# NYXFLOWER/GripNet

Measured on AMD Instinct MI355X. Metric: edges aggregated/sec, GripNet forward on pose-0, higher is better.
Workload: dtype f32

## Files before the change

gripnet_amd/_hip.py:

```python
from __future__ import annotations

import ctypes as C
import operator
import os
import threading

import torch

from ._cache import MISS, VersionedCache

_LIB_PATH = os.environ.get("GN_HIP_LIBRARY") or os.path.join(os.path.dirname(os.path.abspath(__file__)), "lib",
                                                            "libgripnet_hip.so")
_lib = None
_lock = threading.Lock()

GN_OK, GN_ERR_INVALID_ARG, GN_ERR_HIP, GN_ERR_INDEX_RANGE, GN_ERR_UNSUPPORTED, GN_ERR_EDGE_COUNT = range(6)
GN_RGCN_PARTIAL, GN_RGCN_ARITH_FAST, GN_RGCN_BASIS_TRANSPOSED = 1, 4, 64
GN_RGCN_PATH_SHIFT = 8
RGCN_PATHS = {"auto": 0, "pair": 1, "lds": 3, "general": 4, "table": 5}
GN_GEMM_RELU, GN_GEMM_ARITH_FAST, GN_GEMM_B_TRANSPOSED, GN_GEMM_ACCUMULATE, GN_GEMM_A_TRANSPOSED, GN_GEMM_JOIN_BATCH, GN_GEMM_OUT_BF16 = 1, 2, 4, 8, 16, 32, 64
GN_DM_TYPES_SORTED = 1
GN_DM_TYPE_TASKS = 2
ABI_VERSION = 165

_p, _i64, _int, _sz = C.c_void_p, C.c_int64, C.c_int, C.c_size_t

SIGNATURES = {
    "gn_version": (_int, []),
    "gn_last_error": (C.c_char_p, []),
    "gn_time_next_launch": (_int, [_p, _p]),
    "gn_host_scratch_release": (_sz, []),
    "gn_device_blocks_live": (_i64, []),
    "gn_time_launch_pending": (_int, []),
    "gn_gcn_plan_create": (_int, [_p, _p, _p, _i64, _i64, _int, _p, C.POINTER(_p)]),
    "gn_bipartite_plan_create": (_int, [_p, _p, _p, _i64, _i64, _i64, _p, C.POINTER(_p)]),
    "gn_sum_plan_create": (_int, [_p, _p, _p, _i64, _i64, _i64, _p, C.POINTER(_p)]),
    "gn_graph_plan_destroy": (None, [_p]),
    "gn_graph_plan_input_edges": (_i64, [_p]),
    "gn_graph_plan_nnz": (_i64, [_p]),
    "gn_graph_plan_export": (_int, [_p, _p, _p, _p]),
    "gn_graph_aggregate_f32": (_int, [_p, _p, _i64, _i64, _p, _i64, _p, _int, _p, _i64, _p, _p, _p]),
    "gn_split_planes_bytes": (_sz, [_i64, _int]),
    "gn_split_planes_f32": (_int, [_p, _i64, _i64, _i64, _i64, _p, _p]),
    "gn_transform_fusable": (_int, [_i64, _i64]),
    "gn_graph_transform_fusable": (_int, [_p, _i64, _i64]),
    "gn_graph_plan_build_blocked": (_int, [_p, _i64, _p]),
    "gn_graph_plan_blocked_cols": (_i64, [_p]),
    "gn_graph_plan_blocked_gather_kernel": (_int, [_p]),
    "gn_graph_plan_blocked_waves": (_i64, [_p, _p, _i64]),
    "gn_graph_blocked_applicable": (_int, [_p, _p, _i64, _i64, _p, _i64, _p, _p, _i64]),
    "gn_graph_chain_applicable": (_int, [_p, _p, _p, _i64, _i64, _p, _i64, _p, _p, _i64, _p]),
    "gn_graph_aggregate_chain_f32": (_int, [_p, _p, _p, _i64, _i64, _p, _i64, _p, _int, _p, _i64, _p, _p]),
    "gn_graph_gather_chained_f32": (_int, [_p, _p, _i64, _p]),
    "gn_graph_aggregate_tail_f32": (_int, [_p, _p, _i64, _i64, _p, _i64, _p, _int, _p, _i64, _p, _p, _p, _p, _int, _p]),
    "gn_graph_plan_build_transpose": (_int, [_p, _p]),
    "gn_graph_aggregate_t_f32": (_int, [_p, _p, _i64, _i64, _p, _i64, _p]),
    "gn_xtg_wide_supported": (_int, [_i64, _i64, _i64]),
    "gn_gemm_f32": (_int, [_p, _i64, _i64, _p, _i64, _p, _i64, _i64, _p, _i64, _i64, _i64, _i64, _i64, _i64, _p, _int, _p]),
    "gn_gemm_addend_f32": (_int, [_p, _i64, _i64, _p, _i64, _p, _i64, _i64, _p, _i64, _i64, _i64, _i64, _i64, _i64, _p, _p, _i64, _int, _p]),
    "gn_merge_f32": (_int, [_p, _i64, _p, _i64, _p, _i64, _i64, _i64, _int, _p]),
    "gn_softmax_rows_f32": (_int, [_p, _i64, _i64, _i64, _p]),
    "gn_softmax_rows_backward_f32": (_int, [_p, _i64, _p, _i64, _p, _i64, _i64, _i64, _p]),
    "gn_class_scores_f32": (_int, [_p, _i64, _i64, _p, _i64, _p, _i64, _i64, _i64, _int, _p, _i64, _p]),
    "gn_rgcn_plan_create": (_int, [_p, _p, _p, _int, _i64, _i64, _i64, _i64, _i64, _p, C.POINTER(_p)]),
    "gn_rgcn_plan_create_ex": (_int, [_p, _p, _p, _int, _i64, _i64, _i64, _i64, _i64, _int, _p, C.POINTER(_p)]),
    "gn_rgcn_plan_destroy": (None, [_p]),
    "gn_rgcn_plan_input_edges": (_i64, [_p]),
    "gn_rgcn_workspace_bytes": (_sz, [_p, _i64, _i64, _i64, _int]),
    "gn_rgcn_forward_path": (_int, [_p, _i64, _i64, _i64, _int]),
    "gn_rgcn_forward_choice": (_int, [_p, _p, _i64, _i64, _i64, _i64, _int, C.POINTER(_sz)]),
    "gn_cast_bf16": (_int, [_p, _i64, _p, _i64, _i64, _i64, _p]),
    "gn_graph_aggregate_bf16": (_int, [_p, _p, _i64, _i64, _p, _int, _p, _i64, _p, _p]),
    "gn_rgcn_forward_f32": (_int, [_p, _p, _i64, _i64, _p, _p, _i64, _p, _p, _i64, _int, _int, _p, _i64, _p, _p, _p, _sz, _p]),
    "gn_rgcn_finalize_f32": (_int, [_p, _p, _i64, _p, _i64, _i64, _p, _p, _i64, _int, _p, _i64, _p, _p]),
    "gn_distmult_forward_f32": (_int, [_p, _i64, _i64, _i64, _p, _p, _p, _p, _i64, _i64, _i64, _int, _p, _p, _p]),
    "gn_distmult_packed_forward_f32": (_int, [_p, _i64, _i64, _i64, _p, _p, _p, _i64, _i64, _i64, _int, _p, _p, _p]),
    "gn_distmult_plan_create": (_int, [_p, _p, _p, _i64, _i64, _i64, _i64, _p, C.POINTER(_p)]),
    "gn_distmult_plan_destroy": (None, [_p]),
    "gn_distmult_plan_edges": (_i64, [_p]),
    "gn_distmult_plan_forward_f32": (_int, [_p, _p, _i64, _i64, _p, _i64, _int, _p, _p]),
    "gn_distmult_plan_forward_cols_f32": (_int, [_p, _p, _i64, _i64, _i64, _i64, _p, _i64, _int, _p, _p]),
    "gn_xtg_workspace_bytes": (_sz, [_i64, _i64]),
    "gn_xtg_f32": (_int, [_p, _i64, _p, _i64, _i64, _i64, _i64, _p, _i64, _p, _sz, _int, _p]),
    "gn_distmult_backward_workspace_bytes": (_sz, [_i64, _i64, _i64, _i64]),
    "gn_dense_batch_begin": (_int, []),
    "gn_dense_batch_end": (_int, [_p]),
    "gn_distmult_type_tasks_bytes": (_sz, [_i64, _i64]),
# ... 608 lines not shown

    @property
    def nnz(self) -> int:
        return int(load().gn_graph_plan_nnz(self._h))

    def export(self):
        if self._export is None:
            n = self.nnz
            ei = torch.empty((2, n), dtype=torch.int64, device=self.device)
            nrm = torch.empty((n,), dtype=torch.float32, device=self.device)
            check(load().gn_graph_plan_export(self._h, ptr(ei), ptr(nrm), stream_ptr(self.device)))
            self._export = (ei, nrm)
        return self._export

    def __iter__(self):
        return iter(self.export())

    def aggregate(self, xw: torch.Tensor, bias, relu: bool, out: torch.Tensor, side=None, weight=None, planes=None, tail=None):
        sc = side_copy(side)
        pd = None
        if planes is not None:
            pd = planes[0].desc(planes[1], planes[2])
            planes[0].generation += 1
        if tail is not None:
            _call("gn_graph_aggregate_tail_f32", self._h, ptr(xw), ld(xw), xw.shape[1], ptr(weight), weight.shape[1], ptr(bias),
                  int(bool(relu)), ptr(out), ld(out), _ref(sc), _ref(pd), ptr(tail[0]), ptr(tail[1]), 1, stream_ptr(xw.device),
                  tag="gn_graph_aggregate_tail_f32[{}]".format(self.kind))
            return out
        _call("gn_graph_aggregate_f32", self._h, ptr(xw), ld(xw), xw.shape[1], ptr(weight),
              0 if weight is None else weight.shape[1], ptr(bias), int(bool(relu)),
              ptr(out), ld(out), _ref(sc), _ref(pd), stream_ptr(xw.device), tag="gn_graph_aggregate_f32[{}]".format(self.kind))
        return out

    def chain_ok(self, nxt: "GraphPlan", x: torch.Tensor, weight: torch.Tensor, bias, out: torch.Tensor, out_next: torch.Tensor) -> bool:
        return bool(load().gn_graph_chain_applicable(self._h, nxt._h, x.data_ptr(), ld(x), x.shape[1], weight.data_ptr(),
                                                     weight.shape[1], None if bias is None else bias.data_ptr(),
                                                     out.data_ptr(), ld(out), out_next.data_ptr()))

    def aggregate_chain(self, nxt: "GraphPlan", x: torch.Tensor, weight: torch.Tensor, bias, relu: bool, out: torch.Tensor, side=None):
        sc = side_copy(side)
        _call("gn_graph_aggregate_chain_f32", self._h, nxt._h, ptr(x), ld(x), x.shape[1], ptr(weight), weight.shape[1], ptr(bias),
              int(bool(relu)), ptr(out), ld(out), _ref(sc), stream_ptr(x.device))
        return out

    def gather_chained(self, out: torch.Tensor):
        _call("gn_graph_gather_chained_f32", self._h, ptr(out), ld(out), stream_ptr(out.device))
        return out

    def aggregate_bf16(self, xw: torch.Tensor, bias, relu: bool, out: torch.Tensor, side=None):
        if xw.dtype == torch.bfloat16:
            table = xw
        else:
            table = torch.empty(xw.shape, dtype=torch.bfloat16, device=xw.device)
            _call("gn_cast_bf16", ptr(xw), ld(xw), ptr(table), ld(table), xw.shape[0], xw.shape[1], stream_ptr(xw.device))
        sc = side_copy(side)
        _call("gn_graph_aggregate_bf16", self._h, ptr(table), ld(table), xw.shape[1], ptr(bias), int(bool(relu)),
              ptr(out), ld(out), _ref(sc), stream_ptr(xw.device), tag="gn_graph_aggregate_bf16[{}]".format(self.kind))
        return out

    def aggregate_t(self, g: torch.Tensor, out: torch.Tensor):
        if not getattr(self, "_has_t", False):
            check(load().gn_graph_plan_build_transpose(self._h, stream_ptr(g.device)))
            self._has_t = True
        _call("gn_graph_aggregate_t_f32", self._h, ptr(g), ld(g), g.shape[1], ptr(out), ld(out), stream_ptr(g.device))
        return out

# ... 709 lines not shown
```

gripnet_amd/csrc/aggregate.cuh:

```cuda
#pragma once

#include "common.h"

#ifndef GN_AGG_U
#define GN_AGG_U 2
#endif
#ifndef GN_AGG_U_WIDE
#define GN_AGG_U_WIDE 8
#endif
#ifndef GN_AGG_GRID
#define GN_AGG_GRID (256 * 8)
#endif

#ifndef GN_AGG_SHORT_MAX_DEG
#define GN_AGG_SHORT_MAX_DEG 8
#endif
#ifndef GN_AGG_GROUP_MAX_DEG
#define GN_AGG_GROUP_MAX_DEG 48
#endif
#ifndef GN_AGG_GROUP_U
#define GN_AGG_GROUP_U 8
#endif
#ifndef GN_MFMA_U16
#define GN_MFMA_U16 4
// ... 1 lines not shown

namespace gn {

struct AggArgs {
    const int32_t* rowptr;
    const uint32_t* col;
    const float* coef;
    const float* table;
    int64_t ld_table;
    int features;
    const float* rowdiv;
    const float* addend;
    int64_t ld_addend;
    const float* bias;
    int relu;
    float* out;
    int64_t ld_out;
    int rows;
    gn_side_copy side = {nullptr, 0, nullptr, 0, 0, 0, 0};
    gn_split_planes split = {nullptr, 0, 0, 0, 0};
    const uint32_t* ell_col = nullptr;
    const float* ell_coef = nullptr;
    int64_t nnz = -1;
    int64_t table_rows = -1;
    const uint16_t* table_bf16 = nullptr;
};

struct AggTail {
    const float* w;
    const float* b;
    int relu;
};

__device__ __forceinline__ void side_copy_stream(gn_side_copy s, int64_t thread, int64_t n_threads) {
    if (s.dst) {
        const int64_t total = s.rows * s.cols;
        for (int64_t t = thread; t < total; t += n_threads) {
            const int64_t i = t / s.cols, c = t - i * s.cols;
            const float v = s.src[i * s.ld_src + c];
            s.dst[i * s.ld_dst + c] = s.mode ? fabsf(v) : v;
        }
    }
}

inline int lanes_per_row(int64_t units) {
    int lpe = 1;
    while (lpe < units && lpe < kWave) lpe <<= 1;
    return lpe;
}

inline gn_status check_side(const gn_side_copy* side, int64_t rows, gn_side_copy* out) {
    *out = gn_side_copy{nullptr, 0, nullptr, 0, 0, 0, 0};
    if (!side || side->rows == 0 || side->cols == 0) return GN_OK;
    GN_REQUIRE(side->src && side->dst && side->rows > 0 && side->cols > 0, "side copy has a null pointer or a negative size");
    GN_REQUIRE(side->rows <= rows, "side copy has %lld rows, the launch only %lld", (long long)side->rows, (long long)rows);
    GN_REQUIRE(side->ld_src >= side->cols && side->ld_dst >= side->cols, "side copy leading dimension smaller than its row");
    GN_REQUIRE(side->mode == 0 || side->mode == 1, "unknown side copy mode %d", side->mode);
    *out = *side;
    return GN_OK;
}

inline bool transform_fusable(int64_t fin, int64_t fout) {
    if (fast_paths_disabled()) return false;
    return (fout == 16 && (fin == 16 || fin == 32 || fin == 64)) || (fout == 32 && (fin == 32 || fin == 64));
}

inline bool mfma_fusable(int64_t fin, int64_t fout, int64_t rows, int64_t nnz) {
    if (fast_paths_disabled()) return false;
    if (!(fin == 64 || fin == 128) || fout % 16 != 0 || fout < fin || fout > 128) return false;
    return nnz >= 0 && nnz < GN_AGG_GROUP_MAX_DEG * rows && rows >= 4096;
}

inline bool quad_gather_disabled() {
    const char* e = getenv("GN_DISABLE_QUAD");
    return e && e[0] == '1';
}

inline bool transform_takes_quad_kernel(int64_t fin, int64_t fout) { return fin == 16 && fout == 16 && !quad_gather_disabled(); }

inline bool lds_table_disabled() {
    const char* e = getenv("GN_DISABLE_LDS_TABLE");
    return e && e[0] == '1';
}

gn_status launch_aggregate(const AggArgs& a, hipStream_t st);
gn_status launch_aggregate_bf16(const AggArgs& a, int lpe, bool by_group, hipStream_t st);
gn_status launch_aggregate_transform(const AggArgs& a, const float* w, int fout, hipStream_t st);
gn_status launch_aggregate_transform_tail(const AggArgs& a, const float* w, int fout, const AggTail& tail, hipStream_t st);
gn_status launch_aggregate_mfma(const AggArgs& a, const float* w, int fout, hipStream_t st);
gn_status launch_split_planes(const float* src, int64_t ld_src, int64_t rows, int cols, int col0, const gn_split_planes& sp, hipStream_t st);

}
```

gripnet_amd/csrc/aggregate.hip:

```cpp
#include "aggregate.cuh"

#include <type_traits>

namespace gn {
namespace {

typedef float f32x4 __attribute__((ext_vector_type(4)));
typedef uint32_t u32x4 __attribute__((ext_vector_type(4)));

struct RowScalar {
    static constexpr int N = 1;
    static constexpr bool kMean = true;
    typedef float elem;
    typedef float raw;
    static __device__ __forceinline__ const elem* table(const AggArgs& a) { return a.table; }
    static __device__ __forceinline__ raw load(const elem* p) { return *p; }
    static __device__ __forceinline__ void add(float (&acc)[N], float coef, raw r) { acc[0] += coef * r; }
};
struct RowF32 {
    static constexpr int N = 4;
    static constexpr bool kMean = true;
    typedef float elem;
    typedef f32x4 raw;
    static __device__ __forceinline__ const elem* table(const AggArgs& a) { return a.table; }
// ... 176 lines not shown
                vv[u] = __shfl(v, t0 + u, LPE);
                r[u] = typename Row::raw{};
                if (t0 + u < cnt && active) r[u] = Row::load(tab + (int64_t)cc * a.ld_table);
            }
#pragma unroll
            for (int u = 0; u < U; ++u) Row::add(acc, vv[u], r[u]);
        }
    }
}

template <typename Row, int LPE, int U>
__global__ __launch_bounds__(256) void k_aggregate_group(AggArgs a) {
    constexpr int S = kWave / LPE, N = Row::N;
    const int lane = threadIdx.x & 63, slot = lane / LPE, j = lane % LPE;
    const int wave = (int)((blockIdx.x * (int64_t)blockDim.x + threadIdx.x) >> 6);
    const int fcol = N * j;
    const bool active = fcol < a.features;
    side_copy_stream(a.side, blockIdx.x * (int64_t)blockDim.x + threadIdx.x, (int64_t)gridDim.x * blockDim.x);
    const int row = wave * S + slot;
    const bool live = row < a.rows;
    const int begin = live ? a.rowptr[row] : 0, end = live ? a.rowptr[row + 1] : 0;
    float acc[N];
#pragma unroll
    for (int t = 0; t < N; ++t) acc[t] = 0.f;
    gather_group_row<Row, LPE, U>(a, Row::table(a) + fcol, begin, end, j, active, acc);
    if (live && active) finish_row<Row::kMean>(a, row, fcol, acc);
}

template <int CTRL>
__device__ __forceinline__ float tail_bcast(float v) {
    return __int_as_float(__builtin_amdgcn_mov_dpp(__float_as_int(v), CTRL, 0xf, 0xf, true));
}

template <int LPE, int FOUT, bool TAIL>
__device__ __forceinline__ void aggregate_transform(const AggArgs& a, const float* __restrict__ w, const AggTail& tail) {
    constexpr int FIN = 4 * LPE, S = kWave / LPE, G = kWave / FOUT, KPL = FIN / G;
    static_assert(KPL % 4 == 0, "K slice per lane must cover whole float4 groups");
    static_assert(!TAIL || LPE == 16, "the deferred tail transform is the last quad of a 16-lane group");
    const int lane = threadIdx.x & 63;
    const int slot = lane / LPE, j = lane % LPE;
    const int c = lane % FOUT, kq = lane / FOUT;
    const int block = blockIdx.x, n_blocks = gridDim.x;
    const int wave = (int)((block * (int64_t)blockDim.x + threadIdx.x) >> 6);
    const int n_waves = (int)(((int64_t)n_blocks * blockDim.x) >> 6);
    float wreg[KPL];
#pragma unroll
    for (int i = 0; i < KPL; ++i) wreg[i] = w[(kq * KPL + i) * FOUT + c];
    const float bias = a.bias ? a.bias[c] : 0.f;
    f32x4 tw[TAIL ? 16 : 1], tb = (f32x4){0.f, 0.f, 0.f, 0.f};
    if constexpr (TAIL) {
#pragma unroll
        for (int k = 0; k < 16; ++k) tw[k] = *reinterpret_cast<const f32x4*>(tail.w + 16 * k + 4 * (j & 3));
        if (tail.b) tb = *reinterpret_cast<const f32x4*>(tail.b + 4 * (j & 3));
    }

    const int64_t side_total = a.side.dst ? a.side.rows * a.side.cols : 0;
    const int64_t side_t0 = block * (int64_t)blockDim.x + threadIdx.x;
    float side_first = 0.f;
    if (side_t0 < side_total) {
        const int64_t i = side_t0 / a.side.cols, cc = side_t0 - i * a.side.cols;
        side_first = a.side.src[i * a.side.ld_src + cc];
    }
    for (int row = wave; row < a.rows; row += n_waves) {
        int begin, end;
        uint32_t cl0 = 0u;
        float v0 = 0.f;
        if (a.ell_col) {
            cl0 = a.ell_col[(size_t)row * 64 + lane];
            v0 = a.ell_coef[(size_t)row * 64 + lane];
            begin = 0;
            end = __popcll(__ballot(cl0 != 0xffffffffu));
            if (lane >= end) cl0 = 0u;
        } else {
            begin = a.rowptr[row];
            end = a.rowptr[row + 1];
        }
        float acc[4] = {0.f, 0.f, 0.f, 0.f};
        for (int base = begin; base < end; base += kWave) {
            const int mine = base + lane;
            const uint32_t cl = a.ell_col ? cl0 : (mine < end ? a.col[mine] : 0u);
            const float v = a.ell_col ? v0 : (mine < end ? (a.coef ? a.coef[mine] : 1.0f) : 0.f);
            const int cnt = min(kWave, end - base);
            constexpr int IT = kWave / S, UW = LPE >= 16 ? GN_AGG_U_WIDE : GN_AGG_U, U = IT < UW ? IT : UW;
            for (int it0 = 0; it0 * S < cnt; it0 += U) {
                float4 t[U];
                float vv[U];
#pragma unroll
                for (int it = 0; it < U; ++it) {
                    const int idx = (it0 + it) * S + slot;
                    const uint32_t cc = (uint32_t)__shfl((int)cl, idx);
                    vv[it] = __shfl(v, idx);
                    t[it] = make_float4(0.f, 0.f, 0.f, 0.f);
                    if (idx < cnt) t[it] = *reinterpret_cast<const float4*>(a.table + (int64_t)cc * a.ld_table + 4 * j);
                }
                if constexpr (TAIL) {
#pragma unroll
                    for (int it = 0; it < U; ++it) {
                        if ((it0 + it) * S >= cnt) continue;
                        const float g[4] = {t[it].x, t[it].y, t[it].z, t[it].w};
                        f32x4 h = tb;
#pragma unroll
                        for (int cc = 0; cc < 4; ++cc) {
                            h += tail_bcast<0x00>(g[cc]) * tw[cc];
                            h += tail_bcast<0x55>(g[cc]) * tw[4 + cc];
                            h += tail_bcast<0xAA>(g[cc]) * tw[8 + cc];
                            h += tail_bcast<0xFF>(g[cc]) * tw[12 + cc];
                        }
                        if (tail.relu) {
#pragma unroll
                            for (int cc = 0; cc < 4; ++cc) h[cc] = fmaxf(h[cc], 0.f);
                        }
                        if (j >= 12 && (it0 + it) * S + slot < cnt) t[it] = make_float4(h[0], h[1], h[2], h[3]);
                    }
                }
#pragma unroll
                for (int it = 0; it < U; ++it) {
                    acc[0] += vv[it] * t[it].x; acc[1] += vv[it] * t[it].y; acc[2] += vv[it] * t[it].z; acc[3] += vv[it] * t[it].w;
                }
            }
        }
#pragma unroll
        for (int off = LPE; off < kWave; off <<= 1) {
#pragma unroll
            for (int t = 0; t < 4; ++t) acc[t] += __shfl_xor(acc[t], off);
        }
        float part = 0.f;
#pragma unroll
        for (int i = 0; i < KPL; ++i) part += __shfl(acc[i % 4], kq * (KPL / 4) + i / 4) * wreg[i];
#pragma unroll
        for (int off = FOUT; off < kWave; off <<= 1) part += __shfl_xor(part, off);
        if (kq == 0) {
            float val = part + bias;
            if (a.relu) val = fmaxf(val, 0.f);
            a.out[(int64_t)row * a.ld_out + c] = val;
            if (a.split.planes) write_split(a.split, row, a.split.col_main + c, val);
        }
    }
    for (int64_t t = side_t0; t < side_total; t += (int64_t)n_blocks * blockDim.x) {
        const int64_t i = t / a.side.cols, cc = t - i * a.side.cols;
        const float v = t == side_t0 ? side_first : a.side.src[i * a.side.ld_src + cc];
        const float o = a.side.mode ? fabsf(v) : v;
        a.side.dst[i * a.side.ld_dst + cc] = o;
        if (a.split.planes) write_split(a.split, i, a.split.col_side + (int)cc, o);
    }
}

template <int LPE, int FOUT>
__global__ __launch_bounds__(256) void k_aggregate_transform(AggArgs a, const float* __restrict__ w) {
    aggregate_transform<LPE, FOUT, false>(a, w, AggTail{nullptr, nullptr, 0});
}
__global__ __launch_bounds__(256) void k_aggregate_transform_tail(AggArgs a, const float* __restrict__ w, AggTail tail) {
    aggregate_transform<16, 16, true>(a, w, tail);
}


template <int CTRL>
__device__ __forceinline__ int agg_dpp(int x) { return __builtin_amdgcn_mov_dpp(x, CTRL, 0xf, 0xf, true); }
template <int CTRL>
__device__ __forceinline__ float agg_dpp_add(float x) {
    return x + __int_as_float(__builtin_amdgcn_update_dpp(0, __float_as_int(x), CTRL, 0xf, 0xf, false));
}

template <int VPL>
__global__ __launch_bounds__(256) void k_aggregate_transform_q(AggArgs a, const float* __restrict__ w) {
    constexpr int FOUT = 16;
    const int lane = threadIdx.x & 63;
    const int q = lane >> 2, j = lane & 3;
    const int wave = (int)((blockIdx.x * (int64_t)blockDim.x + threadIdx.x) >> 6);
    const int n_waves = (int)(((int64_t)gridDim.x * blockDim.x) >> 6);
    f32x4 wreg[VPL];
#pragma unroll
    for (int v = 0; v < VPL; ++v)
#pragma unroll
        for (int c = 0; c < 4; ++c) wreg[v][c] = w[(16 * v + 4 * j + c) * FOUT + q];
    const float bias = a.bias ? a.bias[q] : 0.f;

    side_copy_stream(a.side, blockIdx.x * (int64_t)blockDim.x + threadIdx.x, (int64_t)gridDim.x * blockDim.x);
    const float* __restrict__ tab = a.table + 4 * j;
    for (int row = wave; row < a.rows; row += n_waves) {
        const int begin = a.rowptr[row], end = a.rowptr[row + 1];
        f32x4 s[VPL];
#pragma unroll
        for (int v = 0; v < VPL; ++v) s[v] = (f32x4){0.f, 0.f, 0.f, 0.f};
        for (int base = begin; base < end; base += kWave) {
            const int mine = base + lane;
// ... 250 lines not shown
}

gn_status launch_aggregate_transform(const AggArgs& a, const float* w, int fout, hipStream_t st) {
    if (a.rows == 0) return GN_OK;
    const int grid = (int)std::min<int64_t>(ceil_div(a.rows, 4), GN_AGG_GRID);
    const int key = a.features * 100 + fout;
    if (key == 1616 && a.ld_table % 4 == 0 && aligned16(a.table) && !quad_gather_disabled()) {
        k_aggregate_transform_q<1><<<grid, 256, 0, st>>>(a, w);
        GN_LAUNCH_CHECK();
        return GN_OK;
    }
    switch (key) {
        case 1616: k_aggregate_transform<4, 16><<<grid, 256, 0, st>>>(a, w); break;
        case 3216: k_aggregate_transform<8, 16><<<grid, 256, 0, st>>>(a, w); break;
        case 6416: k_aggregate_transform<16, 16><<<grid, 256, 0, st>>>(a, w); break;
        case 3232: k_aggregate_transform<8, 32><<<grid, 256, 0, st>>>(a, w); break;
        case 6432: k_aggregate_transform<16, 32><<<grid, 256, 0, st>>>(a, w); break;
        default: return fail(GN_ERR_UNSUPPORTED, "no fused transform for %d -> %d features", a.features, fout);
    }
    GN_LAUNCH_CHECK();
    return GN_OK;
}

gn_status launch_aggregate_transform_tail(const AggArgs& a, const float* w, int fout, const AggTail& tail, hipStream_t st) {
    if (a.features != 64 || fout != 16)
        return fail(GN_ERR_UNSUPPORTED, "the deferred tail transform exists for 64 -> 16 features, got %d -> %d", a.features, fout);
    if (a.rows == 0) return GN_OK;
    const int grid = (int)std::min<int64_t>(ceil_div(a.rows, 4), GN_AGG_GRID);
    k_aggregate_transform_tail<<<grid, 256, 0, st>>>(a, w, tail);
    GN_LAUNCH_CHECK();
    return GN_OK;
}

gn_status launch_aggregate(const AggArgs& a, hipStream_t st) {
    if (a.rows == 0 || a.features == 0) return GN_OK;
    const bool vec = (a.features % 4 == 0) && (a.ld_table % 4 == 0) && (a.ld_out % 4 == 0) && aligned16(a.table) &&
                     aligned16(a.out);
    const int lpe = lanes_per_row(vec ? a.features / 4 : a.features);
    if (vec && lpe >= 4 && lpe <= 16 && a.nnz > 0 && a.nnz < 8 * (int64_t)a.rows && a.rows >= 65536 && !a.coef && !a.rowdiv &&
        !a.addend && !a.bias && !a.relu && !a.side.dst && a.table_rows > 0 &&
        (size_t)a.table_rows * a.features * sizeof(float) <= 128 * 1024 && !fast_paths_disabled() && !lds_table_disabled()) {
        const size_t lds = (size_t)(a.table_rows + 1) * a.features * sizeof(float);
        const int wgs = (int)std::min<int64_t>(256, ceil_div((int64_t)a.rows * lpe, 2 * 1024));
        gn_status ls = GN_OK;
        dispatch_lpe<16, 4>(lpe, [&](auto l) {
            ls = allow_large_lds(reinterpret_cast<const void*>(k_aggregate_lds_table<decltype(l)::value>), 160 * 1024);
            if (ls == GN_OK) k_aggregate_lds_table<decltype(l)::value><<<wgs, 1024, lds, st>>>(a);
        });
        if (ls != GN_OK) return ls;
    } else if (vec && lpe <= 16 && a.nnz >= 0 && a.nnz < GN_AGG_SHORT_MAX_DEG * (int64_t)a.rows && !fast_paths_disabled()) {
        const int sgrid = (int)std::min<int64_t>(ceil_div((int64_t)a.rows * lpe, 256), GN_AGG_GRID);
        dispatch_lpe<16>(lpe, [&](auto l) { k_aggregate_short<decltype(l)::value><<<sgrid, 256, 0, st>>>(a); });
    } else if (vec && lpe <= 32 && a.nnz >= 0 && a.nnz < GN_AGG_GROUP_MAX_DEG * (int64_t)a.rows && !fast_paths_disabled()) {
        launch_group_per_row<RowF32>(a, lpe, st);
    } else if (vec) {
        launch_wave_per_row<RowF32>(a, lpe, st);
    } else {
        launch_wave_per_row<RowScalar>(a, lpe, st);
    }
    GN_LAUNCH_CHECK();
    return GN_OK;
}

gn_status launch_aggregate_bf16(const AggArgs& a, int lpe, bool by_group, hipStream_t st) {
    if (by_group) launch_group_per_row<RowBf16>(a, lpe, st); else launch_wave_per_row<RowBf16>(a, lpe, st);
    GN_LAUNCH_CHECK();
// ... 5 lines not shown
```

gripnet_amd/csrc/graph.hip:

```cpp
#include "aggregate.cuh"

bool gn_blocked_applicable(const gn_graph_plan* plan, const float* x, int64_t ld_x, int64_t fin, const float* w, int64_t fout,
                           const float* bias, const float* out, int64_t ld_out);
gn_status gn_blocked_aggregate(const gn_graph_plan* plan, const float* x, int64_t ld_x, int64_t fin, const float* w,
                               int64_t fout, const float* bias, int relu, float* out, int64_t ld_out,
                               const gn_side_copy& side, hipStream_t st);

static gn::AggArgs forward_args(const gn_graph_plan* plan, const float* xw, int64_t ld_xw, int64_t num_features, const float* bias,
                                int relu, float* out, int64_t ld_out) {
    gn::AggArgs a;
    a.rowptr = plan->rowptr.p;
    a.col = reinterpret_cast<const uint32_t*>(plan->col.p);
    a.coef = plan->plain_ones ? nullptr : plan->coef.p;
    a.table = xw;
    a.ld_table = ld_xw;
    a.features = (int)num_features;
    a.rowdiv = nullptr;
    a.addend = nullptr;
    a.ld_addend = 0;
    a.bias = bias;
    a.relu = relu;
    a.out = out;
    a.ld_out = ld_out;
    a.rows = (int)plan->rows;
// ... 46 lines not shown
                            (long long)num_features, (long long)out_features);
        const bool quad = gn::transform_takes_quad_kernel(num_features, out_features);
        if (planes && planes->planes && !quad) a.split = *planes;
        const gn_status s = gn::launch_aggregate_transform(a, weight, (int)out_features, gn::as_stream(stream));
        return quad ? then_split(s) : s;
    }
    return then_split(gn::launch_aggregate(a, gn::as_stream(stream)));
}

extern "C" gn_status gn_graph_aggregate_tail_f32(const gn_graph_plan* plan, const float* x, int64_t ld_x, int64_t num_features,
                                                 const float* weight, int64_t out_features, const float* bias, int relu,
                                                 float* out, int64_t ld_out, const gn_side_copy* side,
                                                 const gn_split_planes* planes, const float* tail_w, const float* tail_b,
                                                 int tail_relu, void* stream) {
    GN_REQUIRE(plan != nullptr, "plan is null");
    GN_REQUIRE(x && weight && out && tail_w, "a feature or weight pointer is null");
    GN_REQUIRE(ld_x >= num_features && ld_out >= out_features, "leading dimension smaller than the row length");
    if (num_features != 64 || out_features != 16 || gn::fast_paths_disabled() || (ld_x % 4) != 0 || !gn::aligned16(x) ||
        !gn::aligned16(tail_w) || !gn::aligned16(tail_b))
        return gn::fail(GN_ERR_UNSUPPORTED, "the deferred tail transform exists for 64 -> 16 features over 16-byte aligned rows "
                                            "on the wave-per-row kernel, got %lld -> %lld", (long long)num_features,
                        (long long)out_features);
    if (plan->rows == 0) return GN_OK;
    gn::AggArgs a = forward_args(plan, x, ld_x, num_features, bias, relu, out, ld_out);
    gn_status ss = gn::check_side(side, plan->rows, &a.side);
    if (ss != GN_OK) return ss;
    ss = check_planes(planes, plan, out_features, a.side);
    if (ss != GN_OK) return ss;
    if (planes && planes->planes) a.split = *planes;
    return gn::launch_aggregate_transform_tail(a, weight, (int)out_features, gn::AggTail{tail_w, tail_b, tail_relu},
                                               gn::as_stream(stream));
}

extern "C" size_t gn_split_planes_bytes(int64_t rows, int nt) {
    if (rows < 0 || nt < 1) return 0;
    return (size_t)(rows + 1) * 64 * (size_t)((3 * nt + 1) / 2);
}

extern "C" gn_status gn_split_planes_f32(const float* src, int64_t ld_src, int64_t rows, int64_t cols, int64_t col0,
                                         const gn_split_planes* planes, void* stream) {
    GN_REQUIRE(planes && planes->planes, "planes are null");
    GN_REQUIRE(planes->nt >= 1 && planes->nt <= 4 && rows >= 0 && rows <= planes->rows && cols >= 0 && col0 >= 0 &&
                   col0 + cols <= 16 * planes->nt, "split planes do not hold these columns");
    if (rows == 0 || cols == 0) return GN_OK;
    GN_REQUIRE(src && ld_src >= cols, "source matrix is null or its leading dimension too small");
    return gn::launch_split_planes(src, ld_src, rows, (int)cols, (int)col0, *planes, gn::as_stream(stream));
}

extern "C" gn_status gn_graph_aggregate_t_f32(const gn_graph_plan* plan, const float* g, int64_t ld_g,
                                              int64_t num_features, float* out, int64_t ld_out, void* stream) {
    GN_REQUIRE(plan != nullptr, "plan is null");
    GN_REQUIRE(plan->has_transpose, "call gn_graph_plan_build_transpose first");
    GN_REQUIRE(num_features >= 0 && num_features < (1ll << 31), "bad feature count");
    if (plan->table_rows == 0 || num_features == 0) return GN_OK;
    GN_REQUIRE(g && out, "feature pointers are null");
    GN_REQUIRE(ld_g >= num_features && ld_out >= num_features, "leading dimension smaller than the row length");
    gn::AggArgs a;
    a.rowptr = plan->t_rowptr.p;
    a.col = reinterpret_cast<const uint32_t*>(plan->t_col.p);
    a.coef = plan->t_coef.p;
    a.table = g;
    a.ld_table = ld_g;
    a.features = (int)num_features;
    a.rowdiv = nullptr;
    a.addend = nullptr;
    a.ld_addend = 0;
// ... 19 lines not shown
```

gripnet_amd/layers.py:

```python
from __future__ import annotations

import math

import numpy as np
import torch
from torch.nn import Module, Parameter

from . import _hip
from .autograd import AbsSlotFn, GcnConvFn, HalfSumAbsFn, HalfSumDownFn, RgcnConvFn, Slot, SlotsCatFn, cat_slots, recording


def _unslot(out, side):
    if isinstance(out, Slot):
        out = out.view()
    if side is not None and isinstance(side[1], Slot):
        side = (side[0].detach(), side[1].view(), side[2])
    return out, side


class myGCN(Module):

    def __init__(self, in_channels, out_channels, improved=False, cached=False, bias=True, **kwargs):
        super().__init__()
        self.in_channels, self.out_channels = in_channels, out_channels
# ... 305 lines not shown
                hold=lambda: (inter_edge_index, edge_weight, conv.cached_result), post=retag)
        y = self.conv.forward_bipartite(x, inter_edge_index, self.n_target, edge_weight, _relu=if_relu)
        if y.shape[1] == self.target_feat.shape[1]:
            return _hip.merge(y, self.target_feat, 2)
        down = torch.empty_like(y)
        _hip.gemm(self.target_feat, self.target_feat_down, down)
        return _hip.merge(y, down, 3)

    def _cat_planes(self, dev):
        width, planes = self.target_dim + self.target_feat_dim, None
        if width % 16 == 0 and width <= 64 and self.conv.table_storage == "fp32":
            planes = getattr(self, "_planes", None)
            if planes is None or planes.device != dev:
                planes = self._planes = _hip.SplitPlanes(self.n_target, width // 16, dev)
        return planes

    def _infer_cat(self, x, inter_edge_index, edge_weight, if_relu, out):
        dev = x.device
        y, tf = out[:, :self.target_dim], out[:, self.target_dim:]
        planes = self._cat_planes(dev)
        self.conv.forward_bipartite(x, inter_edge_index, self.n_target, edge_weight, _out=y, _relu=if_relu,
                                    _side=(self.target_feat, tf, 1),
                                    _planes=None if planes is None else (planes, 0, self.target_dim))
        if planes is not None and getattr(self.conv, "_planes_written", False):
            planes.tag(out)
        return out


def gene_stack_to_external(gg, gd, gg_edge_index, edge_weight, gd_edge_index, if_relu=True):
    chained = _gene_chain(gg, gd, gg_edge_index, edge_weight, gd_edge_index, if_relu)
    gg.__dict__["_gene_stack_path"] = "separate" if chained is None else "chained"
    if chained is not None:
        return chained
    z = gg(None, gg_edge_index, edge_weight=edge_weight, if_catout=True)
    return gd(z, gd_edge_index, mod="cat", if_relu=if_relu)


def gene_stack_path(gg):
    return gg.__dict__.get("_gene_stack_path")


def _gene_chain(gg, gd, gg_edge_index, edge_weight, gd_edge_index, if_relu):
    if torch.is_grad_enabled() or not isinstance(gg, homoGraph) or not isinstance(gd, interGraph):
        return None
    if gg.multi_relational or not gg.start_graph or len(gg.conv_list) != 2 or not gd.if_one_external:
        return None
    c1, c2, cd = gg.conv_list[0], gg.conv_list[1], gd.conv
    widths = [gg.embedding.shape[1], c1.out_channels, c2.out_channels]
    if (c2.in_channels, c2.out_channels) != (16, 16) or sum(widths) != 64 or (cd.in_channels, cd.out_channels) != (64, 16):
        return None
    if any(c.table_storage != "fp32" or c.arithmetic != "fp32" or not c.weight.is_contiguous() for c in (c1, c2, cd)):
        return None
    if not c1.cached or not c2.cached or c2.bias is None or not gd.target_feat.is_contiguous():
        return None
    _hip.require_gpu(gg.embedding, gg_edge_index, edge_weight, gd_edge_index)
    x = _hip.f32_rows(gg.embedding.detach())
    n, dev = x.shape[0], x.device
    p1, p2 = c1._gcn_plan(gg_edge_index, n, edge_weight), c2._gcn_plan(gg_edge_index, n, edge_weight)
    pd = cd._plan(gd_edge_index, lambda: _hip.GraphPlan.bipartite(gd_edge_index, n, gd.n_target, None))
    out = torch.empty((gd.n_target, gd.target_dim + gd.target_feat_dim), dtype=torch.float32, device=dev)

    def run():
        genes = torch.empty((n, 64), dtype=torch.float32, device=dev)
        s0, s1, s2 = genes[:, :widths[0]], genes[:, widths[0]:widths[0] + 16], genes[:, 48:]
        if not (p1.chain_ok(p2, x, c1.weight, c1.bias, s1, s2) and pd.transform_ok(64, 16, genes)):
            raise _NotChained()
        p1.aggregate_chain(p2, x, c1.weight, c1.bias, True, s1, side=(x, s0, 0))
        p2.gather_chained(s2)
        planes = gd._cat_planes(dev)
        pd.aggregate(genes, cd.bias, if_relu, out[:, :gd.target_dim], (gd.target_feat, out[:, gd.target_dim:], 1),
                     weight=cd.weight, planes=None if planes is None else (planes, 0, gd.target_dim), tail=(c2.weight, c2.bias))
        if planes is not None:
            planes.tag(out)
        return out

    try:
        return _gene_chain_memo(gg, gd, gg_edge_index, edge_weight, gd_edge_index, if_relu, x, out, (c1, c2, cd), (p1, p2, pd), run)
    except _NotChained:
        return None


class _NotChained(Exception):
    """The library does not take the chained launches for these operands."""


def _gene_chain_memo(gg, gd, gg_edge_index, edge_weight, gd_edge_index, if_relu, x, out, convs, plans, run):
    if _hip._recorder is not None:
        return run()
    n, dev = x.shape[0], x.device
    guard = (x.data_ptr(), n, x.stride(0), id(gg_edge_index), gg_edge_index._version, id(edge_weight),
             0 if edge_weight is None else edge_weight._version, id(gd_edge_index), gd_edge_index._version, bool(if_relu), id(gd),
             gd.target_feat.data_ptr(),
             tuple([(id(c.cached_result),) + tuple([0 if p is None else p.data_ptr() for p in c._parameters.values()])
                    for c in convs]),
             _hip.launch_context(dev), _hip.env_stamp())
    memo = gg.__dict__.get("_chain_memo")
    if memo is None:
        memo = gg.__dict__["_chain_memo"] = _hip.CallMemo()

    def retag():
        planes = _hip.SplitPlanes.of(out, out.shape[1] // 16) if out.shape[1] % 16 == 0 else None
        return None if planes is None else planes.rewritten_for
    return memo.run(guard, out, run, drop=(out,), hold=lambda: (gg_edge_index, edge_weight, gd_edge_index, gd) + tuple(plans), post=retag)
```

include/gripnet_hip.h:

```cpp
#ifndef GRIPNET_HIP_H
#define GRIPNET_HIP_H

#include <stddef.h>
#include <stdint.h>

#ifdef __cplusplus
extern "C" {
#endif

#define GN_VERSION 165

#if defined(GN_BUILDING)
#define GN_API __attribute__((visibility("default")))
#else
#define GN_API
#endif

typedef enum gn_status {
    GN_OK = 0,
    GN_ERR_INVALID_ARG = 1,
    GN_ERR_HIP = 2,
    GN_ERR_INDEX_RANGE = 3,
    GN_ERR_UNSUPPORTED = 4,
    GN_ERR_EDGE_COUNT = 5
} gn_status;

typedef struct gn_side_copy {
    const float* src; int64_t ld_src;
    float* dst; int64_t ld_dst;
    int64_t rows, cols;
    int mode;
} gn_side_copy;

typedef struct gn_split_planes {
    void* planes;
    int64_t rows;
    int nt;
    int col_main;
    int col_side;
} gn_split_planes;

typedef struct gn_graph_plan gn_graph_plan;
typedef struct gn_rgcn_plan gn_rgcn_plan;

GN_API int gn_version(void);
GN_API const char* gn_last_error(void);
GN_API int64_t gn_device_blocks_live(void);

GN_API gn_status gn_gcn_plan_create(const int64_t* src, const int64_t* dst, const float* w, int64_t num_edges,
                             int64_t num_nodes, int improved, void* stream, gn_graph_plan** plan);

GN_API gn_status gn_bipartite_plan_create(const int64_t* src, const int64_t* dst, const float* w, int64_t num_edges,
                                   int64_t num_sources, int64_t num_targets, void* stream, gn_graph_plan** plan);

GN_API gn_status gn_sum_plan_create(const int64_t* src, const int64_t* dst, const float* w, int64_t num_edges,
                             int64_t num_sources, int64_t num_targets, void* stream, gn_graph_plan** plan);

GN_API void gn_graph_plan_destroy(gn_graph_plan* plan);
GN_API int64_t gn_graph_plan_input_edges(const gn_graph_plan* plan);
GN_API int64_t gn_graph_plan_nnz(const gn_graph_plan* plan);
GN_API gn_status gn_graph_plan_export(const gn_graph_plan* plan, int64_t* edge_index_out, float* norm_out, void* stream);

GN_API gn_status gn_graph_aggregate_f32(const gn_graph_plan* plan, const float* xw, int64_t ld_xw, int64_t num_features,
                                 const float* weight , int64_t out_features,
                                 const float* bias, int relu, float* out, int64_t ld_out,
                                 const gn_side_copy* side , const gn_split_planes* planes ,
                                 void* stream);
GN_API size_t gn_split_planes_bytes(int64_t rows, int nt);
GN_API gn_status gn_split_planes_f32(const float* src, int64_t ld_src, int64_t rows, int64_t cols, int64_t col0,
                              const gn_split_planes* planes, void* stream);
GN_API int gn_transform_fusable(int64_t in_features, int64_t out_features);
GN_API int gn_graph_transform_fusable(const gn_graph_plan* plan, int64_t in_features, int64_t out_features);

GN_API gn_status gn_graph_plan_build_blocked(gn_graph_plan* plan, int64_t cols, void* stream);
GN_API int64_t gn_graph_plan_blocked_cols(const gn_graph_plan* plan);
GN_API int gn_graph_plan_blocked_gather_kernel(const gn_graph_plan* plan);
GN_API int64_t gn_graph_plan_blocked_waves(const gn_graph_plan* plan, int32_t* host_out, int64_t capacity);
GN_API int gn_graph_blocked_applicable(const gn_graph_plan* plan, const float* x, int64_t ld_x, int64_t num_features,
                                       const float* weight, int64_t out_features, const float* bias, const float* out,
                                       int64_t ld_out);

GN_API int gn_graph_chain_applicable(const gn_graph_plan* plan, const gn_graph_plan* next, const float* x, int64_t ld_x,
                                     int64_t num_features, const float* weight, int64_t out_features, const float* bias,
                                     const float* out, int64_t ld_out, const float* out_next);
GN_API gn_status gn_graph_aggregate_chain_f32(const gn_graph_plan* plan, const gn_graph_plan* next, const float* x, int64_t ld_x,
                                       int64_t num_features, const float* weight, int64_t out_features, const float* bias,
                                       int relu, float* out, int64_t ld_out, const gn_side_copy* side ,
                                       void* stream);
GN_API gn_status gn_graph_gather_chained_f32(const gn_graph_plan* plan, float* out, int64_t ld_out, void* stream);
GN_API gn_status gn_graph_aggregate_tail_f32(const gn_graph_plan* plan, const float* x, int64_t ld_x, int64_t num_features,
                                      const float* weight, int64_t out_features, const float* bias, int relu, float* out,
                                      int64_t ld_out, const gn_side_copy* side ,
                                      const gn_split_planes* planes , const float* tail_w,
                                      const float* tail_b , int tail_relu, void* stream);

GN_API gn_status gn_cast_bf16(const float* src, int64_t ld_src, uint16_t* dst, int64_t ld_dst, int64_t rows, int64_t cols,
                       void* stream);
GN_API gn_status gn_graph_aggregate_bf16(const gn_graph_plan* plan, const uint16_t* table, int64_t ld_table, int64_t num_features,
                                  const float* bias, int relu, float* out, int64_t ld_out,
                                  const gn_side_copy* side , void* stream);

GN_API gn_status gn_graph_plan_build_transpose(gn_graph_plan* plan, void* stream);
GN_API gn_status gn_graph_aggregate_t_f32(const gn_graph_plan* plan, const float* g, int64_t ld_g, int64_t num_features,
                                   float* out, int64_t ld_out, void* stream);

// ... 285 lines not shown
```

Baseline: 65.51 billion.

## Read gene concat input from split embedding and layer tables without materializing

```diff
diff --git a/gripnet_amd/_hip.py b/gripnet_amd/_hip.py
--- a/gripnet_amd/_hip.py
+++ b/gripnet_amd/_hip.py
@@ -21,7 +21,7 @@
 GN_GEMM_RELU, GN_GEMM_ARITH_FAST, GN_GEMM_B_TRANSPOSED, GN_GEMM_ACCUMULATE, GN_GEMM_A_TRANSPOSED, GN_GEMM_JOIN_BATCH, GN_GEMM_OUT_BF16 = 1, 2, 4, 8, 16, 32, 64
 GN_DM_TYPES_SORTED = 1
 GN_DM_TYPE_TASKS = 2
-ABI_VERSION = 165
+ABI_VERSION = 166
 
 _p, _i64, _int, _sz = C.c_void_p, C.c_int64, C.c_int, C.c_size_t
 
@@ -53,6 +53,8 @@
     "gn_graph_aggregate_chain_f32": (_int, [_p, _p, _p, _i64, _i64, _p, _i64, _p, _int, _p, _i64, _p, _p]),
     "gn_graph_gather_chained_f32": (_int, [_p, _p, _i64, _p]),
     "gn_graph_aggregate_tail_f32": (_int, [_p, _p, _i64, _i64, _p, _i64, _p, _int, _p, _i64, _p, _p, _p, _p, _int, _p]),
+    "gn_graph_split_applicable": (_int, [_p, _p, _i64, _i64, _p, _i64, _i64, _i64]),
+    "gn_graph_aggregate_split_f32": (_int, [_p, _p, _i64, _i64, _p, _i64, _i64, _p, _i64, _p, _int, _p, _i64, _p, _p, _p]),
     "gn_graph_plan_build_transpose": (_int, [_p, _p]),
     "gn_graph_aggregate_t_f32": (_int, [_p, _p, _i64, _i64, _p, _i64, _p]),
     "gn_xtg_wide_supported": (_int, [_i64, _i64, _i64]),
@@ -727,6 +729,22 @@
               ptr(out), ld(out), _ref(sc), _ref(pd), stream_ptr(xw.device), tag="gn_graph_aggregate_f32[{}]".format(self.kind))
         return out
 
+    def split_ok(self, head: torch.Tensor, tail: torch.Tensor, fout: int) -> bool:
+        return bool(load().gn_graph_split_applicable(self._h, head.data_ptr(), ld(head), head.shape[1], tail.data_ptr(), ld(tail),
+                                                     head.shape[1] + tail.shape[1], int(fout)))
+
+    def aggregate_split(self, head: torch.Tensor, tail: torch.Tensor, bias, relu: bool, out: torch.Tensor, weight: torch.Tensor,
+                        side=None, planes=None):
+        sc = side_copy(side)
+        pd = None
+        if planes is not None:
+            pd = planes[0].desc(planes[1], planes[2])
+            planes[0].generation += 1
+        _call("gn_graph_aggregate_split_f32", self._h, ptr(head), ld(head), head.shape[1], ptr(tail), ld(tail),
+              head.shape[1] + tail.shape[1], ptr(weight), weight.shape[1], ptr(bias), int(bool(relu)), ptr(out), ld(out), _ref(sc),
+              _ref(pd), stream_ptr(head.device), tag="gn_graph_aggregate_split_f32[{}]".format(self.kind))
+        return out
+
     def chain_ok(self, nxt: "GraphPlan", x: torch.Tensor, weight: torch.Tensor, bias, out: torch.Tensor, out_next: torch.Tensor) -> bool:
         return bool(load().gn_graph_chain_applicable(self._h, nxt._h, x.data_ptr(), ld(x), x.shape[1], weight.data_ptr(),
                                                      weight.shape[1], None if bias is None else bias.data_ptr(),
diff --git a/gripnet_amd/csrc/aggregate.cuh b/gripnet_amd/csrc/aggregate.cuh
--- a/gripnet_amd/csrc/aggregate.cuh
+++ b/gripnet_amd/csrc/aggregate.cuh
@@ -57,6 +57,12 @@
     int relu;
 };
 
+struct AggSplit {
+    const float* tail;
+    uint32_t ld_tail;
+    int head_cols;
+};
+
 __device__ __forceinline__ void side_copy_stream(gn_side_copy s, int64_t thread, int64_t n_threads) {
     if (s.dst) {
         const int64_t total = s.rows * s.cols;
@@ -112,6 +118,9 @@
 gn_status launch_aggregate_bf16(const AggArgs& a, int lpe, bool by_group, hipStream_t st);
 gn_status launch_aggregate_transform(const AggArgs& a, const float* w, int fout, hipStream_t st);
 gn_status launch_aggregate_transform_tail(const AggArgs& a, const float* w, int fout, const AggTail& tail, hipStream_t st);
+const char* split_source_refusal(const float* head, int64_t ld_head, int64_t head_cols, const float* tail, int64_t ld_tail,
+                                 int64_t features, int64_t fout);
+gn_status launch_aggregate_transform_split(const AggArgs& a, const float* w, int fout, const AggSplit& split, hipStream_t st);
 gn_status launch_aggregate_mfma(const AggArgs& a, const float* w, int fout, hipStream_t st);
 gn_status launch_split_planes(const float* src, int64_t ld_src, int64_t rows, int cols, int col0, const gn_split_planes& sp, hipStream_t st);
 
diff --git a/gripnet_amd/csrc/aggregate.hip b/gripnet_amd/csrc/aggregate.hip
--- a/gripnet_amd/csrc/aggregate.hip
+++ b/gripnet_amd/csrc/aggregate.hip
@@ -232,11 +232,13 @@
     return __int_as_float(__builtin_amdgcn_mov_dpp(__float_as_int(v), CTRL, 0xf, 0xf, true));
 }
 
-template <int LPE, int FOUT, bool TAIL>
-__device__ __forceinline__ void aggregate_transform(const AggArgs& a, const float* __restrict__ w, const AggTail& tail) {
+template <int LPE, int FOUT, bool TAIL, bool SPLIT = false>
+__device__ __forceinline__ void aggregate_transform(const AggArgs& a, const float* __restrict__ w, const AggTail& tail,
+                                                    const AggSplit& split = AggSplit{nullptr, 0, 0}) {
     constexpr int FIN = 4 * LPE, S = kWave / LPE, G = kWave / FOUT, KPL = FIN / G;
     static_assert(KPL % 4 == 0, "K slice per lane must cover whole float4 groups");
     static_assert(!TAIL || LPE == 16, "the deferred tail transform is the last quad of a 16-lane group");
+    static_assert(!SPLIT || !TAIL, "a split source has no deferred tail transform");
     const int lane = threadIdx.x & 63;
     const int slot = lane / LPE, j = lane % LPE;
     const int c = lane % FOUT, kq = lane / FOUT;
@@ -260,6 +262,13 @@
     if (side_t0 < side_total) {
         const int64_t i = side_t0 / a.side.cols, cc = side_t0 - i * a.side.cols;
         side_first = a.side.src[i * a.side.ld_src + cc];
+    }
+    const float* __restrict__ src = nullptr;
+    uint32_t src_ld = 0;
+    if constexpr (SPLIT) {
+        const bool in_head = 4 * j < split.head_cols;
+        src = in_head ? a.table + 4 * j : split.tail + (4 * j - split.head_cols);
+        src_ld = in_head ? (uint32_t)a.ld_table : split.ld_tail;
     }
     for (int row = wave; row < a.rows; row += n_waves) {
         int begin, end;
@@ -291,7 +300,11 @@
                     const uint32_t cc = (uint32_t)__shfl((int)cl, idx);
                     vv[it] = __shfl(v, idx);
                     t[it] = make_float4(0.f, 0.f, 0.f, 0.f);
-                    if (idx < cnt) t[it] = *reinterpret_cast<const float4*>(a.table + (int64_t)cc * a.ld_table + 4 * j);
+                    if constexpr (SPLIT) {
+                        if (idx < cnt) t[it] = *reinterpret_cast<const float4*>(src + (uint64_t)cc * src_ld);
+                    } else {
+                        if (idx < cnt) t[it] = *reinterpret_cast<const float4*>(a.table + (int64_t)cc * a.ld_table + 4 * j);
+                    }
                 }
                 if constexpr (TAIL) {
 #pragma unroll
@@ -351,6 +364,10 @@
 }
 __global__ __launch_bounds__(256) void k_aggregate_transform_tail(AggArgs a, const float* __restrict__ w, AggTail tail) {
     aggregate_transform<16, 16, true>(a, w, tail);
+}
+template <int FOUT>
+__global__ __launch_bounds__(256) void k_aggregate_transform_split(AggArgs a, const float* __restrict__ w, AggSplit split) {
+    aggregate_transform<16, FOUT, false, true>(a, w, AggTail{nullptr, nullptr, 0}, split);
 }
 
 
@@ -667,6 +684,28 @@
     return GN_OK;
 }
 
+const char* split_source_refusal(const float* head, int64_t ld_head, int64_t head_cols, const float* tail, int64_t ld_tail,
+                                 int64_t features, int64_t fout) {
+    if (fast_paths_disabled()) return "the wave-per-row transform kernel is switched off (GN_DISABLE_FAST)";
+    if (features != 64 || fout != 16) return "the split source exists for 64 -> 16 features";
+    if (head_cols != 16 && head_cols != 32 && head_cols != 48) return "head_cols must be 16, 32 or 48";
+    if (!head || !tail || !aligned16(head) || !aligned16(tail)) return "both tables must be 16-byte aligned";
+    if (ld_head % 4 != 0 || ld_tail % 4 != 0) return "both leading dimensions must be multiples of 4";
+    if (ld_head < head_cols || ld_tail < features - head_cols) return "a leading dimension is smaller than its table's row";
+    if (ld_head >= (1ll << 31) || ld_tail >= (1ll << 31)) return "a leading dimension does not fit 31 bits";
+    return nullptr;
+}
+
+gn_status launch_aggregate_transform_split(const AggArgs& a, const float* w, int fout, const AggSplit& split, hipStream_t st) {
+    const char* why = split_source_refusal(a.table, a.ld_table, split.head_cols, split.tail, split.ld_tail, a.features, fout);
+    if (why) return fail(GN_ERR_UNSUPPORTED, "split source, %d -> %d features, head %d: %s", a.features, fout, split.head_cols, why);
+    if (a.rows == 0) return GN_OK;
+    const int grid = (int)std::min<int64_t>(ceil_div(a.rows, 4), GN_AGG_GRID);
+    k_aggregate_transform_split<16><<<grid, 256, 0, st>>>(a, w, split);
+    GN_LAUNCH_CHECK();
+    return GN_OK;
+}
+
 gn_status launch_aggregate(const AggArgs& a, hipStream_t st) {
     if (a.rows == 0 || a.features == 0) return GN_OK;
     const bool vec = (a.features % 4 == 0) && (a.ld_table % 4 == 0) && (a.ld_out % 4 == 0) && aligned16(a.table) &&
diff --git a/gripnet_amd/csrc/graph.hip b/gripnet_amd/csrc/graph.hip
--- a/gripnet_amd/csrc/graph.hip
+++ b/gripnet_amd/csrc/graph.hip
@@ -102,6 +102,33 @@
                                                gn::as_stream(stream));
 }
 
+extern "C" int gn_graph_split_applicable(const gn_graph_plan* plan, const float* head, int64_t ld_head, int64_t head_cols,
+                                         const float* tail, int64_t ld_tail, int64_t num_features, int64_t out_features) {
+    return plan && !gn::split_source_refusal(head, ld_head, head_cols, tail, ld_tail, num_features, out_features) ? 1 : 0;
+}
+
+extern "C" gn_status gn_graph_aggregate_split_f32(const gn_graph_plan* plan, const float* head, int64_t ld_head, int64_t head_cols,
+                                                  const float* tail, int64_t ld_tail, int64_t num_features, const float* weight,
+                                                  int64_t out_features, const float* bias, int relu, float* out, int64_t ld_out,
+                                                  const gn_side_copy* side, const gn_split_planes* planes, void* stream) {
+    GN_REQUIRE(plan != nullptr, "plan is null");
+    GN_REQUIRE(weight && out, "a weight or output pointer is null");
+    const char* why = gn::split_source_refusal(head, ld_head, head_cols, tail, ld_tail, num_features, out_features);
+    if (why)
+        return gn::fail(GN_ERR_UNSUPPORTED, "split source, %lld -> %lld features, head %lld: %s", (long long)num_features,
+                        (long long)out_features, (long long)head_cols, why);
+    GN_REQUIRE(ld_out >= out_features, "leading dimension smaller than the row length");
+    if (plan->rows == 0) return GN_OK;
+    gn::AggArgs a = forward_args(plan, head, ld_head, num_features, bias, relu, out, ld_out);
+    gn_status ss = gn::check_side(side, plan->rows, &a.side);
+    if (ss != GN_OK) return ss;
+    ss = check_planes(planes, plan, out_features, a.side);
+    if (ss != GN_OK) return ss;
+    if (planes && planes->planes) a.split = *planes;
+    return gn::launch_aggregate_transform_split(a, weight, (int)out_features, gn::AggSplit{tail, (uint32_t)ld_tail, (int)head_cols},
+                                                gn::as_stream(stream));
+}
+
 extern "C" size_t gn_split_planes_bytes(int64_t rows, int nt) {
     if (rows < 0 || nt < 1) return 0;
     return (size_t)(rows + 1) * 64 * (size_t)((3 * nt + 1) / 2);
diff --git a/gripnet_amd/layers.py b/gripnet_amd/layers.py
--- a/gripnet_amd/layers.py
+++ b/gripnet_amd/layers.py
@@ -361,6 +361,9 @@
     gg.__dict__["_gene_stack_path"] = "separate" if chained is None else "chained"
     if chained is not None:
         return chained
+    split = _gene_split(gg, gd, gg_edge_index, edge_weight, gd_edge_index, if_relu)
+    if split is not None:
+        return split
     z = gg(None, gg_edge_index, edge_weight=edge_weight, if_catout=True)
     return gd(z, gd_edge_index, mod="cat", if_relu=if_relu)
 
@@ -410,10 +413,51 @@
 
 
 class _NotChained(Exception):
-    """The library does not take the chained launches for these operands."""
-
-
-def _gene_chain_memo(gg, gd, gg_edge_index, edge_weight, gd_edge_index, if_relu, x, out, convs, plans, run):
+    """The library does not take the chained (or the split-source) launches for these operands."""
+
+
+def _gene_split(gg, gd, gg_edge_index, edge_weight, gd_edge_index, if_relu):
+    if torch.is_grad_enabled() or not isinstance(gg, homoGraph) or not isinstance(gd, interGraph):
+        return None
+    if gg.multi_relational or not gg.start_graph or len(gg.conv_list) != 2 or not gd.if_one_external:
+        return None
+    c1, c2, cd = gg.conv_list[0], gg.conv_list[1], gd.conv
+    emb = gg.embedding.detach()
+    w0, w1, w2 = emb.shape[1], c1.out_channels, c2.out_channels
+    if w0 not in (16, 32, 48) or w1 % 4 or w2 % 4 or w0 + w1 + w2 != 64 or (cd.in_channels, cd.out_channels) != (64, 16):
+        return None
+    if any(c.table_storage != "fp32" or c.arithmetic != "fp32" or not c.weight.is_contiguous() for c in (c1, c2, cd)):
+        return None
+    if emb.dtype != torch.float32 or not emb.is_contiguous() or emb.data_ptr() % 16 or not gd.target_feat.is_contiguous():
+        return None
+    _hip.require_gpu(emb, gg_edge_index, edge_weight, gd_edge_index)
+    n, dev = emb.shape[0], emb.device
+    p1, p2 = c1._gcn_plan(gg_edge_index, n, edge_weight), c2._gcn_plan(gg_edge_index, n, edge_weight)
+    pd = cd._plan(gd_edge_index, lambda: _hip.GraphPlan.bipartite(gd_edge_index, n, gd.n_target, None))
+    out = torch.empty((gd.n_target, gd.target_dim + gd.target_feat_dim), dtype=torch.float32, device=dev)
+
+    def run():
+        layers = torch.empty((n, w1 + w2), dtype=torch.float32, device=dev)
+        if not pd.split_ok(emb, layers, cd.out_channels):
+            raise _NotChained()
+        h1 = c1._run(p1, emb, n, layers[:, :w1], True, None)
+        c2._run(p2, h1, n, layers[:, w1:], True, None)
+        planes = gd._cat_planes(dev)
+        pd.aggregate_split(emb, layers, cd.bias, if_relu, out[:, :gd.target_dim], cd.weight,
+                           side=(gd.target_feat, out[:, gd.target_dim:], 1),
+                           planes=None if planes is None else (planes, 0, gd.target_dim))
+        if planes is not None:
+            planes.tag(out)
+        return out
+
+    try:
+        return _gene_chain_memo(gg, gd, gg_edge_index, edge_weight, gd_edge_index, if_relu, emb, out, (c1, c2, cd), (p1, p2, pd), run,
+                                slot="_split_memo")
+    except _NotChained:
+        return None
+
+
+def _gene_chain_memo(gg, gd, gg_edge_index, edge_weight, gd_edge_index, if_relu, x, out, convs, plans, run, slot="_chain_memo"):
     if _hip._recorder is not None:
         return run()
     n, dev = x.shape[0], x.device
@@ -423,9 +467,9 @@
              tuple([(id(c.cached_result),) + tuple([0 if p is None else p.data_ptr() for p in c._parameters.values()])
                     for c in convs]),
              _hip.launch_context(dev), _hip.env_stamp())
-    memo = gg.__dict__.get("_chain_memo")
+    memo = gg.__dict__.get(slot)
     if memo is None:
-        memo = gg.__dict__["_chain_memo"] = _hip.CallMemo()
+        memo = gg.__dict__[slot] = _hip.CallMemo()
 
     def retag():
         planes = _hip.SplitPlanes.of(out, out.shape[1] // 16) if out.shape[1] % 16 == 0 else None
diff --git a/include/gripnet_hip.h b/include/gripnet_hip.h
--- a/include/gripnet_hip.h
+++ b/include/gripnet_hip.h
@@ -8,7 +8,7 @@
 extern "C" {
 #endif
 
-#define GN_VERSION 165
+#define GN_VERSION 166
 
 #if defined(GN_BUILDING)
 #define GN_API __attribute__((visibility("default")))
@@ -71,6 +71,14 @@
                               const gn_split_planes* planes, void* stream);
 GN_API int gn_transform_fusable(int64_t in_features, int64_t out_features);
 GN_API int gn_graph_transform_fusable(const gn_graph_plan* plan, int64_t in_features, int64_t out_features);
+
+GN_API int gn_graph_split_applicable(const gn_graph_plan* plan, const float* head, int64_t ld_head, int64_t head_cols,
+                                     const float* tail, int64_t ld_tail, int64_t num_features, int64_t out_features);
+GN_API gn_status gn_graph_aggregate_split_f32(const gn_graph_plan* plan, const float* head, int64_t ld_head, int64_t head_cols,
+                                       const float* tail, int64_t ld_tail, int64_t num_features, const float* weight,
+                                       int64_t out_features, const float* bias, int relu, float* out, int64_t ld_out,
+                                       const gn_side_copy* side , const gn_split_planes* planes ,
+                                       void* stream);
 
 GN_API gn_status gn_graph_plan_build_blocked(gn_graph_plan* plan, int64_t cols, void* stream);
 GN_API int64_t gn_graph_plan_blocked_cols(const gn_graph_plan* plan);
```

Result: faster. 67.00 billion, median of 6 (+2.3%).
